# baryshnikova-lab/safepy

Hardware: AMD Instinct MI355X
Metric: node-attribute enrichments/sec (nodes x attrs x perms), compute_pvalues permutation test (higher is better)
Workload: dtype u1 (bit-sliced integer counts; f64 outputs)

## Files before the change

include/safe_hip.h:

```cpp
#ifndef SAFE_HIP_H
#define SAFE_HIP_H

#include <stddef.h>
#include <stdint.h>

#ifdef __cplusplus
extern "C" {
#endif

#define SAFE_HIP_ABI_VERSION 6

#define SAFE_OK 0
#define SAFE_E_INVALID (-1)
#define SAFE_E_HIP (-2)
#define SAFE_E_NOMEM (-3)
#define SAFE_E_UNSUPPORTED (-4)
#define SAFE_E_VALUE (-5)

#define SAFE_DTYPE_F32 0
#define SAFE_DTYPE_F64 1
#define SAFE_DTYPE_U8 2

#define SAFE_SCORE_SUM 0
#define SAFE_SCORE_ZSCORE 1
// ... 84 lines not shown
                             uint64_t key, safe_perms **out);
int safe_ctx_share_stream(safe_ctx *ctx, const char *name, int local_rank, int local_world, int64_t capacity_bytes);
int safe_ctx_unshare_stream(safe_ctx *ctx);
int safe_perms_create_shared(safe_ctx *ctx, int64_t n, const uint8_t *movable_host, int64_t num_permutations,
                             int has_seed, uint32_t seed, safe_perms **out);
int safe_perms_timing(safe_perms *perms, double *out5);
int safe_perms_twin_stats(safe_perms *perms, int *twin_active, int64_t *chunks, int64_t *chunks_won_by_twin);
int safe_ring_open(const char *name, int local_rank, int local_world, int64_t capacity_bytes, safe_ring **out);
int safe_ring_close(safe_ring *ring);
int safe_ring_begin(safe_ring *ring, int64_t n, int64_t k, int64_t count, uint64_t movable_hash, int64_t slot_bytes);
int safe_ring_publish(safe_ring *ring, int64_t chunk, const void *src_host, size_t bytes);
int safe_ring_fetch(safe_ring *ring, int64_t chunk, void *dst_host, size_t bytes);
int safe_ring_end(safe_ring *ring);
int safe_rng_permutations_host(uint32_t seed, const int64_t *values, int64_t n_items,
                               int64_t count, int64_t *out);

int safe_score(safe_ctx *ctx, safe_nbr *nbr, safe_attr *attr, int score_type,
               int64_t col0, int64_t col1, double *out_dev);

int safe_permtest_counts(safe_ctx *ctx, safe_nbr *nbr, safe_attr *attr, safe_perms *perms,
                         int score_type, int64_t col0, int64_t col1, double *ns_dev,
                         double *counts_neg_dev, double *counts_pos_dev);

int safe_randomization(safe_ctx *ctx, safe_nbr *nbr, safe_attr *attr, safe_perms *perms,
                       int score_type, int sign_mode, double enrichment_threshold,
                       const double *nes_table_host, int64_t col0, int64_t col1,
                       double *ns_dev, double *pvalues_neg_dev, double *pvalues_pos_dev,
                       double *nes_dev, double *nes_binary_dev, double *num_enriched_dev);

int safe_hypergeom(safe_ctx *ctx, safe_nbr *nbr, safe_attr *attr, double enrichment_threshold,
// ... 71 lines not shown
```

safepy_amd/_lib.py:

```python
import ctypes as C
import os

_HERE = os.path.dirname(os.path.abspath(__file__))
LIB_PATH = os.path.join(_HERE, 'libsafe_hip.so')

ABI_VERSION = 6
DTYPE_F32, DTYPE_F64, DTYPE_U8 = 0, 1, 2
SCORE_SUM, SCORE_ZSCORE = 0, 1
SIGN_HIGHEST, SIGN_LOWEST, SIGN_BOTH = 0, 1, 2
E_INVALID, E_HIP, E_NOMEM, E_UNSUPPORTED, E_VALUE = -1, -2, -3, -4, -5


class SafeHipError(RuntimeError):
    def __init__(self, code, message):
        super().__init__('libsafe_hip error %d: %s' % (code, message))
        self.code = code


if not os.path.exists(LIB_PATH):
    raise ImportError(
        'safepy_amd: %s not found. Build it with `python -c "import __graft_entry__ as g; g.build()"` or '
        '`make -C safepy_amd/csrc` (needs hipcc, --offload-arch=gfx950). There is no CPU fallback.' % LIB_PATH)


# ... 62 lines not shown
                                     C.POINTER(C.c_int)]),
    'safe_attr_create_host': (C.c_int, [_vp, _vp, C.c_int, _i64, _i64, _i64, _i64, _pp]),
    'safe_attr_create_dev': (C.c_int, [_vp, _vp, C.c_int, _i64, _i64, _i64, _i64, _pp]),
    'safe_attr_destroy': (C.c_int, [_vp]),
    'safe_attr_reindex': (C.c_int, [_vp, _vp, C.c_int, _i64, _i64, _i64, _i64, _vp, _i64, C.c_double, C.c_int, _vp, _pp]),
    'safe_attr_value_counts': (C.c_int, [_vp, _pi64, _pi64, _pi64, _pi64]),
    'safe_attr_nan_to_zero': (C.c_int, [_vp]),
    'safe_attr_download': (C.c_int, [_vp, _vp]),
    'safe_attr_stats': (C.c_int, [_vp, _pi64, _pi64, _pi64, _pi64]),
    'safe_attr_row_flags': (C.c_int, [_vp, _vp]),
    'safe_attr_set_row_flags': (C.c_int, [_vp, _vp]),
    'safe_perms_create': (C.c_int, [_vp, _i64, _vp, _i64, C.c_int, C.c_uint32, _pp]),
    'safe_perms_destroy': (C.c_int, [_vp]),
    'safe_perms_read': (C.c_int, [_vp, _i64, _i64, _vp]),
    'safe_rng_permutations_host': (C.c_int, [C.c_uint32, _vp, _i64, _i64, _vp]),
    'safe_score': (C.c_int, [_vp, _vp, _vp, C.c_int, _i64, _i64, _vp]),
    'safe_permtest_counts': (C.c_int, [_vp, _vp, _vp, _vp, C.c_int, _i64, _i64, _vp, _vp, _vp]),
    'safe_randomization': (C.c_int, [_vp, _vp, _vp, _vp, C.c_int, C.c_int, C.c_double, _vp, _i64, _i64,
                                     _vp, _vp, _vp, _vp, _vp, _vp]),
    'safe_hypergeom': (C.c_int, [_vp, _vp, _vp, C.c_double, _i64, _i64, _vp, _vp, _vp, _vp]),
    'safe_enriched_components': (C.c_int, [_vp, _i64, _i64, _vp, _vp, _vp, _i64, _vp]),
    'safe_jaccard_condensed': (C.c_int, [_vp, _i64, _i64, _vp, _vp]),
    'safe_fdr_adjust': (C.c_int, [_vp, _i64, _i64, _i64, C.c_int, C.c_double, _vp, _vp, _vp, _vp, _vp]),
    'safe_export_packed_counts': (C.c_int, [_vp, _vp, _i64, _pi64, _pi64, C.POINTER(C.c_int)]),
    'safe_nes_from_packed_counts': (C.c_int, [_vp, _vp, _vp, C.c_int, _i64, _i64, _i64, C.c_int, _vp, _vp]),
    'safe_outputs_from_packed_counts': (C.c_int, [_vp, _vp, _vp, C.c_int, _i64, _i64, _i64, C.c_int, C.c_double, _vp, _vp, _vp, _vp, _vp]),
    'safe_set_exchange_chunks': (C.c_int, [_vp, C.c_int, _i64, _vp, _vp]),
    'safe_packed_chunk_info': (C.c_int, [_vp, C.POINTER(C.c_int), _pi64, _pi64]),
    'safe_export_packed_chunk': (C.c_int, [_vp, C.c_int, _vp, _i64, _vp]),
    'safe_export_packed_chunk_narrow': (C.c_int, [_vp, C.c_int, _vp, _i64, _vp]),
# ... 56 lines not shown
```

safepy_amd/backend.py:

```python
import collections
import ctypes as C
import os

import numpy as np

from . import _lib
from ._lib import lib, check

_SCORE = {'sum': _lib.SCORE_SUM, 'z-score': _lib.SCORE_ZSCORE}
_SIGN = {'highest': _lib.SIGN_HIGHEST, 'lowest': _lib.SIGN_LOWEST, 'both': _lib.SIGN_BOTH}


def _ptr(a):
    return C.c_void_p(a.ctypes.data) if a is not None else None


def _split_off_cores(cpus, n_cores, slot=0):
    by_core = {}
    for c in sorted(cpus):
        try:
            sib = set()
            for part in open('/sys/devices/system/cpu/cpu%d/topology/thread_siblings_list' % c).read().strip().split(','):
                lo, _, hi = part.partition('-')
                sib.update(range(int(lo), int(hi or lo) + 1))
# ... 630 lines not shown


def last_mfma_filter(ctx):
    s, u = C.c_int(), C.c_int64()
    check(lib.safe_last_mfma_filter(ctx.handle, C.byref(s), C.byref(u)))
    return s.value, u.value


def rng_permutations_host(seed, values, count):
    values = np.ascontiguousarray(values, dtype=np.int64)
    out = np.empty((count, values.shape[0]), dtype=np.int64)
    check(lib.safe_rng_permutations_host(int(seed), _ptr(values), values.shape[0], int(count), _ptr(out)))
    return out


def nes_table(num_permutations):
    p = np.arange(num_permutations + 1, dtype=np.float64) / num_permutations
    with np.errstate(divide='ignore'):
        return np.ascontiguousarray(-np.log10(np.where(p == 0, 1 / num_permutations, p)))



def score(ctx, nbr, attr, score_type, out_ptr, col0=0, col1=None):
    col1 = attr.m if col1 is None else col1
    check(lib.safe_score(ctx.handle, nbr.handle, attr.handle, _SCORE[score_type], col0, col1, C.c_void_p(out_ptr)))


def permtest_counts(ctx, nbr, attr, perms, score_type, ns_ptr, neg_ptr, pos_ptr, col0=0, col1=None):
    col1 = attr.m if col1 is None else col1
    check(lib.safe_permtest_counts(ctx.handle, nbr.handle, attr.handle, perms.handle, _SCORE[score_type], col0, col1,
# ... 177 lines not shown
```

safepy_amd/csrc/attr.hip:

```cpp
#include "common.h"

template <typename T>
__device__ __forceinline__ double load_attr(const void *raw, int64_t idx) {
    return static_cast<double>(reinterpret_cast<const T *>(raw)[idx]);
}

template <typename T, int GC>
__global__ __launch_bounds__(256) void k_attr_stats(const void *__restrict__ raw, int64_t n, int64_t m,
                                                    int64_t rs, int64_t cs, unsigned int *__restrict__ row_bits,
                                                    unsigned long long *__restrict__ acc ,
                                                    double *__restrict__ col_sum, unsigned long long *__restrict__ max_abs_bits,
                                                    unsigned int *__restrict__ col_nan, int64_t rows_per_block) {
    extern __shared__ unsigned int s_bits[];
    constexpr int RL = 256 / GC;
    const int cx = GC == 1 ? 0 : (threadIdx.x & (GC - 1));
    const int ry = GC == 1 ? threadIdx.x : (threadIdx.x / GC);
    const int lane = threadIdx.x & 63;
    const int64_t j = static_cast<int64_t>(blockIdx.x) * GC + cx;
    const int64_t n_words = (n + 31) / 32;
    __shared__ double s_sum[256];
    __shared__ double s_max[256];
    __shared__ unsigned int s_nan[256], s_other[256], s_nonint[256];
    const int64_t r_begin = static_cast<int64_t>(blockIdx.y) * rows_per_block;
    const int64_t r_end = r_begin + rows_per_block < n ? r_begin + rows_per_block : n;
// ... 310 lines not shown
                       reinterpret_cast<unsigned long long *>(flags + tail_off));
    SAFE_HIP_CHECK(hipGetLastError());
    void *pinned = nullptr;
    SAFE_TRY(ctx_pinned(ctx, flag_bytes, &pinned));
    SAFE_HIP_CHECK(hipMemcpyAsync(pinned, flags, flag_bytes, hipMemcpyDeviceToHost, ctx->stream));
    SAFE_HIP_CHECK(safe_stream_sync(ctx->stream));
    const uint8_t *h_flags = static_cast<const uint8_t *>(pinned);
    unsigned long long h_acc[4];
    memcpy(h_acc, h_flags + tail_off, sizeof(h_acc));
    attr->n_other = static_cast<int64_t>(h_acc[0]);
    attr->max_nan_col = static_cast<int64_t>(h_acc[1]);
    attr->n_non_integer = static_cast<int64_t>(h_acc[2]);
    double mx;
    memcpy(&mx, &h_acc[3], sizeof(double));
    attr->max_abs = mx;
    if (!attr->flags_ready) {
        if (attr->row_flags) ctx_block_free(ctx, attr->row_flags, flag_bytes);
        attr->row_flags = flags;
        attr->flags_ready = true;
        int64_t cnt = 0;
        for (int64_t i = 0; i < n; ++i) cnt += h_flags[i] != 0;
        attr->n_rows_with_value = cnt;
        attr->h_row_flags.assign(h_flags, h_flags + n);
    } else {
        ctx_block_free(ctx, flags, flag_bytes);
    }
    attr->stats_ready = true;
    return SAFE_OK;
}

// ... 264 lines not shown
```

safepy_amd/csrc/common.h:

```cpp
#pragma once
#include <hip/hip_runtime.h>

#include <algorithm>
#include <cstdarg>
#include <cmath>
#include <cstdint>
#include <cstdio>
#include <cstdlib>
#include <cstring>
#include <condition_variable>
#include <mutex>
#include <atomic>
#include <string>
#include <thread>
#include <vector>

#include "safe_hip.h"

#define SAFE_WAVE 64
#define SAFE_PAD_U16 0xFFFFu

void safe_set_error(const char *fmt, ...);
void safe_trace(const char *what);

// ... 59 lines not shown
    int num_cu = 0;
    int64_t hbm_bytes = 0;
    char arch[64] = {0};
    hipEvent_t t0 = nullptr, t1 = nullptr;
    hipEvent_t k0 = nullptr, k1 = nullptr;
    KernelStat last_kernel;
    int last_slices = 0;
    void *diag_prof = nullptr;
    int last_core_slices = 0;
    int64_t last_undecided = 0;
    struct safe_perms *perm_cache = nullptr;
    struct PermRing *ring = nullptr;
    const unsigned int *packed_counts = nullptr;
    int64_t packed_n_pad = 0, packed_m = 0, packed_perms = 0;
    int packed_layout = -1;
    static constexpr int XC_MAX = 8;
    int xc_want = 0;
    int64_t xc_cols = 0;
    void (*xc_callback)(void *) = nullptr;
    void *xc_user = nullptr;
    int xc_made = 0;
    int64_t xc_bounds[XC_MAX + 1] = {};
    int64_t xc_tail_perms = 0;
    hipEvent_t xc_events[XC_MAX] = {};
    std::vector<double> nes_tab_host;
    void *pinned = nullptr;
    size_t pinned_bytes = 0;
    static constexpr int D2H_SLOTS = 8;
    static constexpr size_t D2H_SLOT_BYTES = size_t(4) << 20;
    void *d2h_ring = nullptr;
// ... 71 lines not shown
    int64_t bs_groups = 0;
    int64_t bs_blocks = 0;
    int64_t bs_pieces = 0;
    int64_t bs_src = 0;
    int32_t *bs_order = nullptr;
    int32_t *bs_rowmap = nullptr;
    int32_t *bs_rowcnt = nullptr;
    int32_t *bs_grpmax = nullptr;
    uint4 *bs_bits4p = nullptr;
    int64_t bs_max_group_blocks = 0;
    int32_t *bs_ptr = nullptr;
    int32_t *bs_kb = nullptr;
    uint32_t *bs_bits = nullptr;
    std::vector<int32_t> h_bs_ptr;
    std::vector<int32_t> h_bs_rowmap;
    std::vector<int2> counts_tasks;
    int32_t counts_qoff[9] = {0};
    int64_t counts_tasks_grp = -1;
};

struct HypLookup {
    const int32_t *nid;
    const int32_t *kid;
    const double2 *tab;
    int64_t n_kid, xs;
    double p_cut;
    double *dummy;
    double *pvalues_pos, *nes, *nes_binary;
    unsigned int *enriched;
    unsigned int *cnt16;
// ... 30 lines not shown
    double nes_threshold;
    int sign_mode;
    int mode;
    int64_t ld;
};

struct safe_attr {
    safe_ctx *ctx = nullptr;
    int64_t n = 0, m = 0;
    int dtype = SAFE_DTYPE_F64;
    int64_t row_stride = 0, col_stride = 0;
    const void *raw = nullptr;
    bool owns_raw = false;
    uint8_t *row_flags = nullptr;
    std::vector<uint8_t> h_row_flags;
    bool flags_ready = false;
    bool stats_ready = false;
    int64_t n_other = 0, max_nan_col = 0, n_rows_with_value = 0, n_non_integer = 0;
    double *col_sum = nullptr;
    double max_abs = 0.0;
    int32_t *sup_ptr = nullptr;
    int32_t *sup_row = nullptr;
    int64_t n_ones = 0;
    std::vector<int32_t> h_sup_ptr;
};

struct DrawStream;

struct safe_perms {
    safe_ctx *ctx = nullptr;
// ... 45 lines not shown
    uint16_t *inverse_t = nullptr;
    int64_t inv_stride = 0;
    bool from_table = false;
    bool device_gen = false;
    int32_t *d_movpos = nullptr;
    struct PermRing *ring = nullptr;
    bool ring_consumer = false;
    double t_created_s = 0.0, draw_busy_ms = 0.0, drawn_all_ms = 0.0, enqueued_all_ms = 0.0, ring_wait_ms = 0.0;
};

static inline int64_t ceil_div(int64_t a, int64_t b) { return (a + b - 1) / b; }

int safe_attr_prepare(safe_attr *attr);
int nbr_finalize_from_bits(safe_nbr *nbr);
int nbr_build_transpose(safe_nbr *nbr);
int attr_build_support(safe_attr *attr);
int perms_build_inverse(safe_perms *perms);
int perms_generate_until(safe_perms *perms, int64_t upto);
std::vector<int64_t> perms_stage_plan(int64_t count);
static inline std::vector<int64_t> perm_launch_starts(const safe_perms *perms, int64_t *span, int merge = 1) {
    const int64_t P = perms->count;
    std::vector<int64_t> starts;
    int64_t uniform = 0;
    if (const char *e = getenv("SAFE_HIP_BITS_SPAN")) uniform = std::max<int64_t>(16, atoll(e));
    if (uniform > 0) {
        for (int64_t p = 0; p < P; p += uniform) starts.push_back(p);
    } else {
        const std::vector<int64_t> &plan = perms->stages;
        const int64_t nc = static_cast<int64_t>(plan.size()) - 1;
        for (int64_t c = 0; c < nc; ++c)
// ... 24 lines not shown
```

safepy_amd/csrc/enrich.hip:

```cpp
#include <algorithm>
#include <cmath>
#include <numeric>

#include "common.h"

template <typename T, int BN, int PLANES>
__global__ __launch_bounds__(256) void k_tile_prep(const void *__restrict__ raw, int64_t n, int64_t rs, int64_t cs,
                                                   int64_t col0, int64_t mloc, int64_t n_tiles,
                                                   double *__restrict__ bt) {
    const int64_t idx = static_cast<int64_t>(blockIdx.x) * 256 + threadIdx.x;
    const int64_t total = n_tiles * (n + 1) * BN;
    if (idx >= total) return;
    const int c = static_cast<int>(idx % BN);
    const int64_t row = (idx / BN) % (n + 1);
    const int64_t tile = idx / (static_cast<int64_t>(BN) * (n + 1));
    const int64_t j = tile * BN + c;
    double v = 0.0, v2 = 0.0, nn = 0.0;
    if (row < n && j < mloc) {
        const T x = reinterpret_cast<const T *>(raw)[row * rs + (col0 + j) * cs];
        if (x == x) {
            v = static_cast<double>(x);
            v2 = static_cast<double>(static_cast<T>(x * x));
            nn = 1.0;
        }
// ... 2248 lines not shown
    double ph[5][3] = {}, cls_n[5] = {0, 0, 0, 0, 0};
    for (unsigned int i = 0; i < cnt; ++i) {
        const double nb = static_cast<double>(rec[8 * i + 3] >> 32);
        const int c = nb <= 1 ? 0 : nb <= 7 ? 1 : nb <= 31 ? 2 : nb <= 63 ? 3 : 4;
        ph[c][0] += static_cast<double>(rec[8 * i + 4] - rec[8 * i + 1]);
        ph[c][1] += static_cast<double>(rec[8 * i + 5] - rec[8 * i + 4]);
        ph[c][2] += static_cast<double>(rec[8 * i + 2] - rec[8 * i + 5]);
        cls_n[c] += 1.0;
    }
    for (int c = 0; c < 5; ++c)
        if (cls_work[c] > 0)
            fprintf(stderr, "[blk trace]   slices of %-12s: %.3g block-iterations, %.0f clocks each; %.0f wave-tasks: table %.1f | counting %.1f | flush %.1f kclk each\n",
                    names[c], cls_work[c], cls_busy[c] / cls_work[c], cls_n[c], ph[c][0] / cls_n[c] / 1e3, ph[c][1] / cls_n[c] / 1e3, ph[c][2] / cls_n[c] / 1e3);
}

static int launch_bits(safe_ctx *ctx, safe_nbr *nbr, safe_attr *attr, safe_perms *perms, int64_t col0, int64_t col1,
                       const PermOut &out) {
    const int64_t n = nbr->n, mloc = col1 - col0, n_wg = ceil_div(mloc, 64), P = perms->count;
    const BitsForm form = bits_form(n, nbr->max_count, nbr->sell_col2 != nullptr, 160 * 1024);
    SAFE_REQUIRE(form.kind != BITS_NONE, "launch_bits: no bit-sliced form for %lld nodes with neighborhoods of up to %lld members",
                 static_cast<long long>(n), static_cast<long long>(nbr->max_count));
    const bool blk = form.kind == BITS_BLK, half = form.kind == BITS_PRE32;
    const int wv = blk ? 4 : 16;
    const int id_shift = blk ? 3 : half ? 0 : 1;
    const int64_t n_wgt = half ? 2 * n_wg : n_wg;
    safe_trace("launch_bits: enter");
    uint2 *d_bits = nullptr;
    SAFE_TRY(ctx_scratch(ctx, 1, static_cast<size_t>(n_wg) * (n + 1) * sizeof(uint2), reinterpret_cast<void **>(&d_bits)));
    launch_bits_prep(ctx, attr, col0, mloc, n_wg, d_bits);
    safe_trace("launch_bits: prep launched");
    int64_t span = 1;
    const std::vector<int64_t> starts = perm_launch_starts(perms, &span);
    int64_t n_major = static_cast<int64_t>(starts.size()) - 1, p_split = P, xc_wpc = 0;
    int xc_k = 0;
// ... 189 lines not shown
            const uint16_t *ids_c = d_ids[c % NS];
            void *args[] = {(void *)&n, (void *)&ids_c, (void *)&entries_pad, (void *)&nbr->sell_row, (void *)&nbr->slice_off,
                            (void *)&nbr->slice_width, (void *)&nbr->sell_col2, (void *)&nbr->n_slices, (void *)&d_bits, (void *)&n_tasks,
                            (void *)&d_tasks, (void *)&p_base, (void *)&p_limit, (void *)&queue_c, (void *)&mloc, (void *)&d_gl,
                            (void *)&n_pad, (void *)&out.ns};
            SAFE_HIP_CHECK(hipLaunchKernel(kfn, dim3(grid), dim3(1024), args, lds_T, ks));
        }
        SAFE_HIP_CHECK(hipGetLastError());
        SAFE_HIP_CHECK(hipEventRecord(ev[2 * c + 1], ks));
    }
    ctx->packed_counts = d_gl;
    ctx->packed_n_pad = n_pad;
    ctx->packed_m = mloc;
    ctx->packed_perms = P;
    ctx->packed_layout = 0;
    SAFE_REQUIRE(xc_rc == SAFE_OK, "launch_bits: recording a column chunk's event failed");
    if (n_tail) {
        ctx->xc_made = static_cast<int>(n_tail);
        ctx->xc_tail_perms = tail_span;
        for (int64_t k = 0; k <= n_tail; ++k) ctx->xc_bounds[k] = std::min<int64_t>(k * ctx->xc_cols, mloc);
        ctx->xc_bounds[n_tail] = mloc;
        safe_trace("launch_bits: column chunks enqueued");
        if (ctx->xc_callback) ctx->xc_callback(ctx->xc_user);
    }
    for (int b = 1; b < NS; ++b) {
        SAFE_HIP_CHECK(hipEventRecord(plain[b], kstreams[b]));
        SAFE_HIP_CHECK(hipStreamWaitEvent(ctx->stream, plain[b], 0));
    }
    SAFE_TRY(enrich_finalize_counts(ctx, d_gl, n_pad, nbr->sell_row, mloc, P, out, nullptr));
    SAFE_HIP_CHECK(hipGetLastError());
// ... 358 lines not shown
                 (long long)ctx->packed_perms);
    *c0 = std::min<int64_t>(chunk * ctx->xc_cols, ctx->packed_m);
    *c1 = chunk + 1 == ctx->xc_want ? ctx->packed_m : std::min<int64_t>((chunk + 1) * ctx->xc_cols, ctx->packed_m);
    const int64_t need = (*c1 - *c0) * (narrow ? ctx->packed_n_pad / 8 * 5 : ctx->packed_n_pad);
    SAFE_REQUIRE(capacity >= need, "%s: buffer holds %lld %s, %lld needed", fn, (long long)capacity, narrow ? "words" : "counters", (long long)need);
    SAFE_HIP_CHECK(hipSetDevice(ctx->device));
    *s = stream ? static_cast<hipStream_t>(stream) : ctx->stream;
    if (ctx->xc_made > 0) {
        SAFE_REQUIRE(ctx->xc_made == ctx->xc_want && ctx->xc_bounds[chunk] == *c0 && ctx->xc_bounds[chunk + 1] == *c1,
                     "%s: the call's chunks are not the armed ones", fn);
        SAFE_HIP_CHECK(hipStreamWaitEvent(*s, ctx->xc_events[chunk], 0));
    }
    return SAFE_OK;
}

extern "C" {

int safe_score(safe_ctx *ctx, safe_nbr *nbr, safe_attr *attr, int score_type, int64_t col0, int64_t col1,
               double *out_dev) {
    SAFE_REQUIRE(ctx && out_dev, "safe_score: NULL argument");
    SAFE_TRY(check_cols(nbr, attr, col0, col1, "safe_score"));
    SAFE_REQUIRE(score_type == SAFE_SCORE_SUM || score_type == SAFE_SCORE_ZSCORE, "safe_score: bad score_type %d", score_type);
    SAFE_HIP_CHECK(hipSetDevice(ctx->device));
    const bool z = score_type == SAFE_SCORE_ZSCORE;
    const CountsRoute route = z ? CountsRoute{} : counts_route(route_switches(), nbr, attr);
    if (route.bits) {
        if (route.mfma) {
            HypLookup hl{};
            hl.pvalues_pos = out_dev;
            SAFE_TRY(launch_mfma_counts(ctx, nbr, attr, col0, col1, hl));
// ... 200 lines not shown
    }
    return SAFE_OK;
}

int safe_export_packed_counts(safe_ctx *ctx, uint32_t *dst_dev, int64_t capacity, int64_t *n_pad, int64_t *m,
                              int *layout) {
    SAFE_REQUIRE(ctx && n_pad && m && layout, "safe_export_packed_counts: NULL argument");
    *layout = ctx->packed_layout;
    *n_pad = ctx->packed_layout >= 0 ? ctx->packed_n_pad : 0;
    *m = ctx->packed_layout >= 0 ? ctx->packed_m : 0;
    if (!dst_dev || ctx->packed_layout < 0) return SAFE_OK;
    const int64_t count = ctx->packed_n_pad * ctx->packed_m;
    SAFE_REQUIRE(capacity >= count, "safe_export_packed_counts: buffer holds %lld counters, %lld needed", (long long)capacity,
                 (long long)count);
    SAFE_HIP_CHECK(hipSetDevice(ctx->device));
    SAFE_HIP_CHECK(hipMemcpyAsync(dst_dev, ctx->packed_counts, static_cast<size_t>(count) * sizeof(uint32_t),
                                  hipMemcpyDeviceToDevice, ctx->stream));
    return SAFE_OK;
}

int safe_outputs_from_packed_counts(safe_ctx *ctx, safe_nbr *nbr, const uint32_t *counts_dev, int layout, int64_t n_pad, int64_t m,
                                    int64_t num_permutations, int sign_mode, double enrichment_threshold,
                                    const double *nes_table_host, double *pvalues_neg_dev, double *pvalues_pos_dev,
                                    double *nes_dev, double *nes_binary_dev) {
    SAFE_REQUIRE(ctx && nbr && counts_dev, "safe_outputs_from_packed_counts: NULL argument");
    SAFE_REQUIRE(pvalues_neg_dev || pvalues_pos_dev || nes_dev || nes_binary_dev, "safe_outputs_from_packed_counts: no output requested");
    SAFE_REQUIRE(layout == 0 || layout == 1, "safe_outputs_from_packed_counts: bad layout %d", layout);
    SAFE_REQUIRE(sign_mode >= SAFE_SIGN_HIGHEST && sign_mode <= SAFE_SIGN_BOTH, "safe_outputs_from_packed_counts: bad sign_mode %d", sign_mode);
    SAFE_REQUIRE(num_permutations >= 1 && num_permutations <= 65535 && m >= 1, "safe_outputs_from_packed_counts: bad sizes");
    SAFE_REQUIRE(enrichment_threshold > 0.0 || !nes_binary_dev, "safe_outputs_from_packed_counts: enrichment_threshold must be positive");
    const int32_t *rowmap = layout == 0 ? nbr->sell_row : nbr->bs_rowmap;
    const int64_t want_pad = layout == 0 ? nbr->n_slices * 64 : nbr->bs_groups * 256;
// ... 27 lines not shown
int safe_packed_chunk_info(safe_ctx *ctx, int *chunks, int64_t *bounds, int64_t *tail_permutations) {
    SAFE_REQUIRE(ctx && chunks, "safe_packed_chunk_info: NULL argument");
    const int made = ctx->packed_layout == 0 ? ctx->xc_made : 0;
    *chunks = made;
    if (bounds)
        for (int k = 0; k <= made; ++k) bounds[k] = ctx->xc_bounds[k];
    if (tail_permutations) *tail_permutations = made ? ctx->xc_tail_perms : 0;
    return SAFE_OK;
}

int safe_export_packed_chunk(safe_ctx *ctx, int chunk, uint32_t *dst_dev, int64_t capacity, void *stream) {
    int64_t c0 = 0, c1 = 0;
    hipStream_t s = nullptr;
    SAFE_TRY(packed_chunk_prepare(ctx, chunk, dst_dev, capacity, false, stream, &c0, &c1, &s));
    const int64_t cells = (c1 - c0) * ctx->packed_n_pad;
    if (cells)
        SAFE_HIP_CHECK(hipMemcpyAsync(dst_dev, ctx->packed_counts + c0 * ctx->packed_n_pad, static_cast<size_t>(cells) * sizeof(uint32_t),
                                      hipMemcpyDeviceToDevice, s));
    if (capacity > cells)
        SAFE_HIP_CHECK(hipMemsetAsync(dst_dev + cells, 0, static_cast<size_t>(capacity - cells) * sizeof(uint32_t), s));
    return SAFE_OK;
}

__global__ __launch_bounds__(256) void k_pack_counts20(const unsigned int *__restrict__ counts, int64_t n_pad, int64_t cols,
                                                       unsigned int *__restrict__ dst) {
    const int64_t half = n_pad / 2, idx = static_cast<int64_t>(blockIdx.x) * 256 + threadIdx.x;
    if (idx >= cols * half) return;
    const int64_t c = idx / half, i = idx % half;
    const uint2 v = *reinterpret_cast<const uint2 *>(counts + c * n_pad + 2 * i);
    const unsigned long long x0 = ((v.x >> 16) << 10) | (v.x & 0x3FFu), x1 = ((v.y >> 16) << 10) | (v.y & 0x3FFu);
    const unsigned long long x = x0 | (x1 << 20);
    unsigned int *col = dst + c * (n_pad / 8 * 5);
    col[i] = static_cast<unsigned int>(x);
    reinterpret_cast<unsigned char *>(col + half)[i] = static_cast<unsigned char>(x >> 32);
}

int safe_export_packed_chunk_narrow(safe_ctx *ctx, int chunk, uint32_t *dst_dev, int64_t capacity_words, void *stream) {
    int64_t c0 = 0, c1 = 0;
    hipStream_t s = nullptr;
    SAFE_TRY(packed_chunk_prepare(ctx, chunk, dst_dev, capacity_words, true, stream, &c0, &c1, &s));
    const int64_t words = (c1 - c0) * (ctx->packed_n_pad / 8 * 5);
    if (words) {
        const int64_t pairs = (c1 - c0) * (ctx->packed_n_pad / 2);
        hipLaunchKernelGGL(k_pack_counts20, dim3(static_cast<unsigned int>(ceil_div(pairs, 256))), dim3(256), 0, s,
                           ctx->packed_counts + c0 * ctx->packed_n_pad, ctx->packed_n_pad, c1 - c0, dst_dev);
        SAFE_HIP_CHECK(hipGetLastError());
    }
    if (capacity_words > words)
        SAFE_HIP_CHECK(hipMemsetAsync(dst_dev + words, 0, static_cast<size_t>(capacity_words - words) * sizeof(uint32_t), s));
    return SAFE_OK;
}

int safe_outputs_from_packed_slabs(safe_ctx *ctx, safe_nbr *nbr, const uint32_t *slabs_dev, int layout, int64_t n_pad, int n_slabs,
                                   int64_t slab_stride, const int64_t *slab_cols, const int64_t *out_col0, int64_t m_total,
                                   int64_t num_permutations, int sign_mode, double enrichment_threshold, const double *nes_table_host,
                                   double *pvalues_neg_dev, double *pvalues_pos_dev, double *nes_dev, double *nes_binary_dev,
                                   void *stream) {
    SAFE_REQUIRE(ctx && nbr && slabs_dev && slab_cols && out_col0 && n_slabs >= 1, "safe_outputs_from_packed_slabs: NULL argument");
    SAFE_REQUIRE(pvalues_neg_dev || pvalues_pos_dev || nes_dev || nes_binary_dev, "safe_outputs_from_packed_slabs: no output requested");
    const bool pk20 = (layout & SAFE_PACKED_NARROW) != 0;
// ... 54 lines not shown
```

safepy_amd/csrc/nbr.hip:

```cpp
#include <algorithm>
#include <cmath>
#include <numeric>

#include "common.h"

static double squared_threshold(double nr) {
    if (!(nr > 0.0)) return 0.0;
    if (std::isinf(nr)) return nr;
    double c = nr * nr;
    if (std::isinf(c)) return c;
    while (c > 0.0 && std::sqrt(c) >= nr) c = std::nextafter(c, 0.0);
    while (std::sqrt(c) < nr) c = std::nextafter(c, INFINITY);
    return c;
}

__global__ __launch_bounds__(256) void k_euclid_bits(const double *__restrict__ xy, int64_t n, double thr_sq,
                                                     uint64_t *__restrict__ bits, int64_t words) {
    __shared__ double sx[64], sy[64];
    const int64_t w = blockIdx.x;
    const int64_t i = static_cast<int64_t>(blockIdx.y) * 256 + threadIdx.x;
    const int64_t j0 = w * 64;
    if (threadIdx.x < 64) {
        const int64_t j = j0 + threadIdx.x;
        sx[threadIdx.x] = j < n ? xy[2 * j] : 0.0;
// ... 282 lines not shown
    (void)hipFree(nbr->bits);
    (void)hipFree(nbr->row_ptr);
    (void)hipFree(nbr->col);
    (void)hipFree(nbr->sell_row);
    (void)hipFree(nbr->sell_pos);
    (void)hipFree(nbr->slice_off);
    (void)hipFree(nbr->slice_width);
    (void)hipFree(nbr->sell_col);
    (void)hipFree(nbr->sell_col2);
    (void)hipFree(nbr->sell_col2b);
    (void)hipFree(nbr->dist);
    (void)hipFree(nbr->at_ptr);
    (void)hipFree(nbr->at_col);
    nbr_free_blocks(nbr);
    if (nbr->bits_plan_pinned) (void)hipHostFree(nbr->bits_plan_pinned);
    delete nbr;
}

static int nbr_new(safe_ctx *ctx, int64_t n, safe_nbr **out) {
    SAFE_REQUIRE(n >= 1 && n < (1ll << 31) - 64, "neighborhood size n=%lld out of range", (long long)n);
    safe_nbr *nbr = new safe_nbr();
    nbr->ctx = ctx;
    nbr->n = n;
    nbr->words = ceil_div(n, 64);
    int rc = dev_alloc(&nbr->bits, static_cast<size_t>(n) * nbr->words);
    if (rc != SAFE_OK) {
        nbr_free(nbr);
        return rc;
    }
    *out = nbr;
    return SAFE_OK;
// ... 11 lines not shown
                                  ctx->stream));
    SAFE_HIP_CHECK(safe_stream_sync(ctx->stream));
    (void)hipFree(d_count);

    std::vector<int32_t> row_ptr(n + 1, 0);
    int64_t nnz = 0, max_count = 0;
    for (int64_t i = 0; i < n; ++i) {
        nnz += nbr->h_row_count[i];
        max_count = std::max<int64_t>(max_count, nbr->h_row_count[i]);
        SAFE_REQUIRE(nnz < (1ll << 31), "membership has too many entries for int32 CSR offsets");
        row_ptr[i + 1] = static_cast<int32_t>(nnz);
    }
    nbr->nnz = nnz;
    nbr->max_count = max_count;

    std::vector<int32_t> order(n);
    std::iota(order.begin(), order.end(), 0);
    std::stable_sort(order.begin(), order.end(), [&](int32_t a, int32_t b) {
        return nbr->h_row_count[a] > nbr->h_row_count[b];
    });
    nbr->n_slices = ceil_div(n, 64);
    std::vector<int32_t> sell_row(nbr->n_slices * 64, -1);
    std::copy(order.begin(), order.end(), sell_row.begin());
    std::vector<int32_t> sell_pos(n);
    for (int64_t t = 0; t < n; ++t) sell_pos[order[t]] = static_cast<int32_t>(t);
    nbr->h_slice_width.assign(nbr->n_slices, 0);
    nbr->h_slice_off.assign(nbr->n_slices + 1, 0);
    for (int64_t s = 0; s < nbr->n_slices; ++s) {
        int32_t wdt = nbr->h_row_count[order[s * 64]];
        wdt = (wdt + 7) & ~7;
        nbr->h_slice_width[s] = wdt;
        nbr->h_slice_off[s + 1] = nbr->h_slice_off[s] + static_cast<int64_t>(wdt) * 64;
    }
    nbr->sell_entries = nbr->h_slice_off[nbr->n_slices];

    SAFE_TRY(dev_alloc(&nbr->row_ptr, n + 1));
    SAFE_TRY(dev_alloc(&nbr->col, nnz));
    SAFE_TRY(dev_alloc(&nbr->sell_row, nbr->n_slices * 64));
    SAFE_TRY(dev_alloc(&nbr->sell_pos, n));
    SAFE_HIP_CHECK(hipMemcpyAsync(nbr->sell_pos, sell_pos.data(), n * sizeof(int32_t), hipMemcpyHostToDevice, ctx->stream));
    SAFE_TRY(dev_alloc(&nbr->slice_off, nbr->n_slices + 1));
    SAFE_TRY(dev_alloc(&nbr->slice_width, nbr->n_slices));
    SAFE_TRY(dev_alloc(&nbr->sell_col, nbr->sell_entries));
    SAFE_HIP_CHECK(hipMemcpyAsync(nbr->row_ptr, row_ptr.data(), (n + 1) * sizeof(int32_t), hipMemcpyHostToDevice,
                                  ctx->stream));
    SAFE_HIP_CHECK(hipMemcpyAsync(nbr->sell_row, sell_row.data(), sell_row.size() * sizeof(int32_t),
                                  hipMemcpyHostToDevice, ctx->stream));
    SAFE_HIP_CHECK(hipMemcpyAsync(nbr->slice_off, nbr->h_slice_off.data(), (nbr->n_slices + 1) * sizeof(int64_t),
                                  hipMemcpyHostToDevice, ctx->stream));
    SAFE_HIP_CHECK(hipMemcpyAsync(nbr->slice_width, nbr->h_slice_width.data(), nbr->n_slices * sizeof(int32_t),
                                  hipMemcpyHostToDevice, ctx->stream));
    hipLaunchKernelGGL(k_fill_csr, dim3(ceil_div(n * 64, 256)), dim3(256), 0, ctx->stream, nbr->bits, n, nbr->words,
                       nbr->row_ptr, nbr->col);
    hipLaunchKernelGGL(k_fill_sell, dim3(nbr->n_slices), dim3(64), 0, ctx->stream, nbr->row_ptr, nbr->col,
                       nbr->sell_row, nbr->slice_off, nbr->slice_width, nbr->n_slices, static_cast<int32_t>(n),
                       nbr->sell_col);
    if (n < 32768) {
        const int64_t total = nbr->sell_entries + 1024;
        SAFE_TRY(dev_alloc(&nbr->sell_col2, total));
        hipLaunchKernelGGL(k_sell_scale16, dim3(ceil_div(total, 256)), dim3(256), 0, ctx->stream, nbr->sell_col,
                           nbr->sell_entries, total, static_cast<uint32_t>(2 * n), nbr->sell_col2);
        SAFE_TRY(dev_alloc(&nbr->sell_col2b, total));
        hipLaunchKernelGGL(k_sell_blocked16, dim3(nbr->n_slices + 1), dim3(256), 0, ctx->stream, nbr->sell_col, nbr->slice_off,
                           nbr->slice_width, nbr->n_slices, nbr->sell_entries, total, static_cast<uint32_t>(2 * n),
                           nbr->sell_col2b);
    }
    SAFE_HIP_CHECK(hipGetLastError());
    SAFE_HIP_CHECK(safe_stream_sync(ctx->stream));
    return SAFE_OK;
}

int nbr_build_transpose(safe_nbr *nbr) {
    if (nbr->at_ptr) return SAFE_OK;
    safe_ctx *ctx = nbr->ctx;
    const int64_t n = nbr->n, nnz = nbr->nnz;
    int32_t *d_cnt = nullptr;
    SAFE_TRY(dev_alloc(&d_cnt, n));
    SAFE_HIP_CHECK(hipMemsetAsync(d_cnt, 0, n * sizeof(int32_t), ctx->stream));
    if (nnz) hipLaunchKernelGGL(k_count_cols, dim3(ceil_div(nnz, 256)), dim3(256), 0, ctx->stream, nbr->col, nnz, d_cnt);
    std::vector<int32_t> cnt(n), ptr(n + 1, 0);
    SAFE_HIP_CHECK(hipMemcpyAsync(cnt.data(), d_cnt, n * sizeof(int32_t), hipMemcpyDeviceToHost, ctx->stream));
    SAFE_HIP_CHECK(safe_stream_sync(ctx->stream));
    for (int64_t k = 0; k < n; ++k) ptr[k + 1] = ptr[k] + cnt[k];
// ... 303 lines not shown
    return SAFE_OK;
}

int safe_nbr_csr(safe_nbr *nbr, int32_t *row_ptr_host, int32_t *col_host) {
    SAFE_REQUIRE(nbr && row_ptr_host && col_host, "safe_nbr_csr: NULL argument");
    safe_ctx *ctx = nbr->ctx;
    SAFE_HIP_CHECK(hipSetDevice(ctx->device));
    SAFE_HIP_CHECK(hipMemcpyAsync(row_ptr_host, nbr->row_ptr, (nbr->n + 1) * sizeof(int32_t), hipMemcpyDeviceToHost,
                                  ctx->stream));
    if (nbr->nnz)
        SAFE_HIP_CHECK(hipMemcpyAsync(col_host, nbr->col, nbr->nnz * sizeof(int32_t), hipMemcpyDeviceToHost, ctx->stream));
    SAFE_HIP_CHECK(safe_stream_sync(ctx->stream));
    return SAFE_OK;
}

int safe_nbr_distances(safe_nbr *nbr, double *out_host) {
    SAFE_REQUIRE(nbr && out_host, "safe_nbr_distances: NULL argument");
    SAFE_REQUIRE(nbr->dist != nullptr, "safe_nbr_distances: handle was built without keep_distances");
    safe_ctx *ctx = nbr->ctx;
    SAFE_HIP_CHECK(hipSetDevice(ctx->device));
    SAFE_HIP_CHECK(hipMemcpyAsync(out_host, nbr->dist, nbr->n * nbr->n * sizeof(double), hipMemcpyDeviceToHost,
                                  ctx->stream));
    SAFE_HIP_CHECK(safe_stream_sync(ctx->stream));
    return SAFE_OK;
}

}
```

Before: 5582 billion.

## Drop neighbor entries of rows without attribute values from bit-sliced permutation lists

Builds a filtered SELL neighborhood structure that removes columns for nodes which are neither movable under the permutation nor carry attribute values. Since those nodes contribute zero, the bit-sliced permutation kernel can scan shorter neighbor lists. The filtered slice order differs from the original, so exported counts go through a remap kernel, and the pack-to-20-bit path gathers through the remap. The filtered structure is cached per drop mask; the cost is a one-time host rebuild and an extra indirect gather on export.

Measured after the change: 5709 billion (median of 6 runs). +2.3%, better.

```diff
diff --git a/include/safe_hip.h b/include/safe_hip.h
--- a/include/safe_hip.h
+++ b/include/safe_hip.h
@@ -122,6 +122,8 @@
 int safe_ring_end(safe_ring *ring);
 int safe_rng_permutations_host(uint32_t seed, const int64_t *values, int64_t n_items,
                                int64_t count, int64_t *out);
+int safe_sell_lists_host(int64_t n, const int32_t *row_ptr, const int32_t *col, const uint8_t *drop, int64_t *entries,
+                         int32_t *row_ptr_out, int32_t *col_out, int32_t *sell_row_out);
 
 int safe_score(safe_ctx *ctx, safe_nbr *nbr, safe_attr *attr, int score_type,
                int64_t col0, int64_t col1, double *out_dev);
diff --git a/safepy_amd/_lib.py b/safepy_amd/_lib.py
--- a/safepy_amd/_lib.py
+++ b/safepy_amd/_lib.py
@@ -100,6 +100,7 @@
     'safe_perms_destroy': (C.c_int, [_vp]),
     'safe_perms_read': (C.c_int, [_vp, _i64, _i64, _vp]),
     'safe_rng_permutations_host': (C.c_int, [C.c_uint32, _vp, _i64, _i64, _vp]),
+    'safe_sell_lists_host': (C.c_int, [_i64, _vp, _vp, _vp, _pi64, _vp, _vp, _vp]),
     'safe_score': (C.c_int, [_vp, _vp, _vp, C.c_int, _i64, _i64, _vp]),
     'safe_permtest_counts': (C.c_int, [_vp, _vp, _vp, _vp, C.c_int, _i64, _i64, _vp, _vp, _vp]),
     'safe_randomization': (C.c_int, [_vp, _vp, _vp, _vp, C.c_int, C.c_int, C.c_double, _vp, _i64, _i64,
diff --git a/safepy_amd/backend.py b/safepy_amd/backend.py
--- a/safepy_amd/backend.py
+++ b/safepy_amd/backend.py
@@ -668,6 +668,20 @@
     return out
 
 
+def sell_lists_host(row_ptr, col, drop=None):
+    row_ptr = np.ascontiguousarray(row_ptr, dtype=np.int32)
+    col = np.ascontiguousarray(col, dtype=np.int32)
+    n = row_ptr.shape[0] - 1
+    drop = None if drop is None else np.ascontiguousarray(drop, dtype=np.uint8)
+    entries = C.c_int64()
+    ptr_out = np.empty(n + 1, dtype=np.int32)
+    col_out = np.empty(max(col.shape[0], 1), dtype=np.int32)
+    sell_row = np.empty(-(-n // 64) * 64, dtype=np.int32)
+    check(lib.safe_sell_lists_host(n, _ptr(row_ptr), _ptr(col), _ptr(drop), C.byref(entries), _ptr(ptr_out), _ptr(col_out),
+                                   _ptr(sell_row)))
+    return {'entries': entries.value, 'row_ptr': ptr_out, 'col': col_out[:ptr_out[-1]], 'sell_row': sell_row}
+
+
 def nes_table(num_permutations):
     p = np.arange(num_permutations + 1, dtype=np.float64) / num_permutations
     with np.errstate(divide='ignore'):
diff --git a/safepy_amd/csrc/attr.hip b/safepy_amd/csrc/attr.hip
--- a/safepy_amd/csrc/attr.hip
+++ b/safepy_amd/csrc/attr.hip
@@ -348,6 +348,7 @@
     double mx;
     memcpy(&mx, &h_acc[3], sizeof(double));
     attr->max_abs = mx;
+    attr->h_local_flags.assign(h_flags, h_flags + n);
     if (!attr->flags_ready) {
         if (attr->row_flags) ctx_block_free(ctx, attr->row_flags, flag_bytes);
         attr->row_flags = flags;
diff --git a/safepy_amd/csrc/common.h b/safepy_amd/csrc/common.h
--- a/safepy_amd/csrc/common.h
+++ b/safepy_amd/csrc/common.h
@@ -97,6 +97,7 @@
     const unsigned int *packed_counts = nullptr;
     int64_t packed_n_pad = 0, packed_m = 0, packed_perms = 0;
     int packed_layout = -1;
+    const int32_t *packed_remap = nullptr;
     static constexpr int XC_MAX = 8;
     int xc_want = 0;
     int64_t xc_cols = 0;
@@ -198,6 +199,9 @@
     uint32_t *bs_bits = nullptr;
     std::vector<int32_t> h_bs_ptr;
     std::vector<int32_t> h_bs_rowmap;
+    safe_nbr *movable_lists = nullptr;
+    std::vector<uint8_t> movable_drop;
+    int32_t *movable_remap = nullptr;
     std::vector<int2> counts_tasks;
     int32_t counts_qoff[9] = {0};
     int64_t counts_tasks_grp = -1;
@@ -258,6 +262,7 @@
     bool owns_raw = false;
     uint8_t *row_flags = nullptr;
     std::vector<uint8_t> h_row_flags;
+    std::vector<uint8_t> h_local_flags;
     bool flags_ready = false;
     bool stats_ready = false;
     int64_t n_other = 0, max_nan_col = 0, n_rows_with_value = 0, n_non_integer = 0;
@@ -333,6 +338,7 @@
 int safe_attr_prepare(safe_attr *attr);
 int nbr_finalize_from_bits(safe_nbr *nbr);
 int nbr_build_transpose(safe_nbr *nbr);
+int nbr_movable_lists(safe_nbr *nbr, const std::vector<uint8_t> &drop, safe_nbr **out);
 int attr_build_support(safe_attr *attr);
 int perms_build_inverse(safe_perms *perms);
 int perms_generate_until(safe_perms *perms, int64_t upto);
diff --git a/safepy_amd/csrc/enrich.hip b/safepy_amd/csrc/enrich.hip
--- a/safepy_amd/csrc/enrich.hip
+++ b/safepy_amd/csrc/enrich.hip
@@ -2286,10 +2286,24 @@
                     names[c], cls_work[c], cls_busy[c] / cls_work[c], cls_n[c], ph[c][0] / cls_n[c] / 1e3, ph[c][1] / cls_n[c] / 1e3, ph[c][2] / cls_n[c] / 1e3);
 }
 
-static int launch_bits(safe_ctx *ctx, safe_nbr *nbr, safe_attr *attr, safe_perms *perms, int64_t col0, int64_t col1,
+static int bits_lists(safe_nbr *nbr, safe_attr *attr, const safe_perms *perms, safe_nbr **out) {
+    *out = nbr;
+    const int64_t n = nbr->n;
+    if (perms->from_table || perms->n != n || perms->k == n || static_cast<int64_t>(perms->h_movable.size()) != perms->k) return SAFE_OK;
+    SAFE_TRY(safe_attr_prepare(attr));
+    if (static_cast<int64_t>(attr->h_local_flags.size()) != n) return SAFE_OK;
+    std::vector<uint8_t> drop(n);
+    for (int64_t i = 0; i < n; ++i) drop[i] = attr->h_local_flags[i] ? 0 : 1;
+    for (const int32_t r : perms->h_movable) drop[r] = 0;
+    return nbr_movable_lists(nbr, drop, out);
+}
+
+static int launch_bits(safe_ctx *ctx, safe_nbr *nbr_full, safe_attr *attr, safe_perms *perms, int64_t col0, int64_t col1,
                        const PermOut &out) {
+    safe_nbr *nbr = nullptr;
+    SAFE_TRY(bits_lists(nbr_full, attr, perms, &nbr));
     const int64_t n = nbr->n, mloc = col1 - col0, n_wg = ceil_div(mloc, 64), P = perms->count;
-    const BitsForm form = bits_form(n, nbr->max_count, nbr->sell_col2 != nullptr, 160 * 1024);
+    const BitsForm form = bits_form(n, nbr_full->max_count, nbr_full->sell_col2 != nullptr, 160 * 1024);
     SAFE_REQUIRE(form.kind != BITS_NONE, "launch_bits: no bit-sliced form for %lld nodes with neighborhoods of up to %lld members",
                  static_cast<long long>(n), static_cast<long long>(nbr->max_count));
     const bool blk = form.kind == BITS_BLK, half = form.kind == BITS_PRE32;
@@ -2509,6 +2523,7 @@
     ctx->packed_m = mloc;
     ctx->packed_perms = P;
     ctx->packed_layout = 0;
+    ctx->packed_remap = nbr != nbr_full ? nbr->movable_remap : nullptr;
     SAFE_REQUIRE(xc_rc == SAFE_OK, "launch_bits: recording a column chunk's event failed");
     if (n_tail) {
         ctx->xc_made = static_cast<int>(n_tail);
@@ -2897,6 +2912,26 @@
     return SAFE_OK;
 }
 
+__global__ __launch_bounds__(256) void k_counts_remap(const unsigned int *__restrict__ counts, const int32_t *__restrict__ remap,
+                                                      int64_t n_pad, int64_t cols, unsigned int *__restrict__ dst) {
+    const int64_t idx = static_cast<int64_t>(blockIdx.x) * 256 + threadIdx.x;
+    if (idx >= cols * n_pad) return;
+    dst[idx] = counts[(idx / n_pad) * n_pad + remap[idx % n_pad]];
+}
+
+static int copy_packed_columns(safe_ctx *ctx, int64_t c0, int64_t c1, uint32_t *dst_dev, hipStream_t s) {
+    const int64_t cells = (c1 - c0) * ctx->packed_n_pad;
+    const unsigned int *src = ctx->packed_counts + c0 * ctx->packed_n_pad;
+    if (ctx->packed_layout == 0 && ctx->packed_remap) {
+        hipLaunchKernelGGL(k_counts_remap, dim3(static_cast<unsigned int>(ceil_div(cells, 256))), dim3(256), 0, s, src, ctx->packed_remap,
+                           ctx->packed_n_pad, c1 - c0, dst_dev);
+        SAFE_HIP_CHECK(hipGetLastError());
+    } else {
+        SAFE_HIP_CHECK(hipMemcpyAsync(dst_dev, src, static_cast<size_t>(cells) * sizeof(uint32_t), hipMemcpyDeviceToDevice, s));
+    }
+    return SAFE_OK;
+}
+
 extern "C" {
 
 int safe_score(safe_ctx *ctx, safe_nbr *nbr, safe_attr *attr, int score_type, int64_t col0, int64_t col1,
@@ -3127,8 +3162,7 @@
     SAFE_REQUIRE(capacity >= count, "safe_export_packed_counts: buffer holds %lld counters, %lld needed", (long long)capacity,
                  (long long)count);
     SAFE_HIP_CHECK(hipSetDevice(ctx->device));
-    SAFE_HIP_CHECK(hipMemcpyAsync(dst_dev, ctx->packed_counts, static_cast<size_t>(count) * sizeof(uint32_t),
-                                  hipMemcpyDeviceToDevice, ctx->stream));
+    SAFE_TRY(copy_packed_columns(ctx, 0, ctx->packed_m, dst_dev, ctx->stream));
     return SAFE_OK;
 }
 
@@ -3186,20 +3220,19 @@
     hipStream_t s = nullptr;
     SAFE_TRY(packed_chunk_prepare(ctx, chunk, dst_dev, capacity, false, stream, &c0, &c1, &s));
     const int64_t cells = (c1 - c0) * ctx->packed_n_pad;
-    if (cells)
-        SAFE_HIP_CHECK(hipMemcpyAsync(dst_dev, ctx->packed_counts + c0 * ctx->packed_n_pad, static_cast<size_t>(cells) * sizeof(uint32_t),
-                                      hipMemcpyDeviceToDevice, s));
+    if (cells) SAFE_TRY(copy_packed_columns(ctx, c0, c1, dst_dev, s));
     if (capacity > cells)
         SAFE_HIP_CHECK(hipMemsetAsync(dst_dev + cells, 0, static_cast<size_t>(capacity - cells) * sizeof(uint32_t), s));
     return SAFE_OK;
 }
 
-__global__ __launch_bounds__(256) void k_pack_counts20(const unsigned int *__restrict__ counts, int64_t n_pad, int64_t cols,
-                                                       unsigned int *__restrict__ dst) {
+__global__ __launch_bounds__(256) void k_pack_counts20(const unsigned int *__restrict__ counts, const int32_t *__restrict__ remap,
+                                                       int64_t n_pad, int64_t cols, unsigned int *__restrict__ dst) {
     const int64_t half = n_pad / 2, idx = static_cast<int64_t>(blockIdx.x) * 256 + threadIdx.x;
     if (idx >= cols * half) return;
     const int64_t c = idx / half, i = idx % half;
-    const uint2 v = *reinterpret_cast<const uint2 *>(counts + c * n_pad + 2 * i);
+    const unsigned int *col_in = counts + c * n_pad;
+    const uint2 v = remap ? make_uint2(col_in[remap[2 * i]], col_in[remap[2 * i + 1]]) : *reinterpret_cast<const uint2 *>(col_in + 2 * i);
     const unsigned long long x0 = ((v.x >> 16) << 10) | (v.x & 0x3FFu), x1 = ((v.y >> 16) << 10) | (v.y & 0x3FFu);
     const unsigned long long x = x0 | (x1 << 20);
     unsigned int *col = dst + c * (n_pad / 8 * 5);
@@ -3215,7 +3248,8 @@
     if (words) {
         const int64_t pairs = (c1 - c0) * (ctx->packed_n_pad / 2);
         hipLaunchKernelGGL(k_pack_counts20, dim3(static_cast<unsigned int>(ceil_div(pairs, 256))), dim3(256), 0, s,
-                           ctx->packed_counts + c0 * ctx->packed_n_pad, ctx->packed_n_pad, c1 - c0, dst_dev);
+                           ctx->packed_counts + c0 * ctx->packed_n_pad, ctx->packed_layout == 0 ? ctx->packed_remap : nullptr,
+                           ctx->packed_n_pad, c1 - c0, dst_dev);
         SAFE_HIP_CHECK(hipGetLastError());
     }
     if (capacity_words > words)
diff --git a/safepy_amd/csrc/nbr.hip b/safepy_amd/csrc/nbr.hip
--- a/safepy_amd/csrc/nbr.hip
+++ b/safepy_amd/csrc/nbr.hip
@@ -320,7 +320,77 @@
     (void)hipFree(nbr->at_col);
     nbr_free_blocks(nbr);
     if (nbr->bits_plan_pinned) (void)hipHostFree(nbr->bits_plan_pinned);
+    (void)hipFree(nbr->movable_remap);
+    nbr_free(nbr->movable_lists);
     delete nbr;
+}
+
+static void sell_slices(const std::vector<int32_t> &count, std::vector<int32_t> &sell_row, std::vector<int32_t> &sell_pos,
+                        std::vector<int32_t> &slice_width, std::vector<int64_t> &slice_off) {
+    const int64_t n = static_cast<int64_t>(count.size()), n_slices = ceil_div(n, 64);
+    std::vector<int32_t> order(n);
+    std::iota(order.begin(), order.end(), 0);
+    std::stable_sort(order.begin(), order.end(), [&](int32_t a, int32_t b) { return count[a] > count[b]; });
+    sell_row.assign(n_slices * 64, -1);
+    std::copy(order.begin(), order.end(), sell_row.begin());
+    sell_pos.resize(n);
+    for (int64_t t = 0; t < n; ++t) sell_pos[order[t]] = static_cast<int32_t>(t);
+    slice_width.assign(n_slices, 0);
+    slice_off.assign(n_slices + 1, 0);
+    for (int64_t s = 0; s < n_slices; ++s) {
+        const int32_t wdt = (count[order[s * 64]] + 7) & ~7;
+        slice_width[s] = wdt;
+        slice_off[s + 1] = slice_off[s] + static_cast<int64_t>(wdt) * 64;
+    }
+}
+
+static void csr_without_rows(int64_t n, const int32_t *row_ptr, const int32_t *col, const uint8_t *drop, std::vector<int32_t> &out_ptr,
+                             std::vector<int32_t> &out_col) {
+    out_ptr.assign(n + 1, 0);
+    out_col.clear();
+    out_col.reserve(row_ptr[n]);
+    for (int64_t i = 0; i < n; ++i) {
+        for (int32_t e = row_ptr[i]; e < row_ptr[i + 1]; ++e)
+            if (!drop[col[e]]) out_col.push_back(col[e]);
+        out_ptr[i + 1] = static_cast<int32_t>(out_col.size());
+    }
+}
+
+static int nbr_build_sell(safe_nbr *nbr) {
+    safe_ctx *ctx = nbr->ctx;
+    const int64_t n = nbr->n;
+    std::vector<int32_t> sell_row, sell_pos;
+    sell_slices(nbr->h_row_count, sell_row, sell_pos, nbr->h_slice_width, nbr->h_slice_off);
+    nbr->n_slices = ceil_div(n, 64);
+    nbr->sell_entries = nbr->h_slice_off[nbr->n_slices];
+    SAFE_TRY(dev_alloc(&nbr->sell_row, nbr->n_slices * 64));
+    SAFE_TRY(dev_alloc(&nbr->sell_pos, n));
+    SAFE_HIP_CHECK(hipMemcpyAsync(nbr->sell_pos, sell_pos.data(), n * sizeof(int32_t), hipMemcpyHostToDevice, ctx->stream));
+    SAFE_TRY(dev_alloc(&nbr->slice_off, nbr->n_slices + 1));
+    SAFE_TRY(dev_alloc(&nbr->slice_width, nbr->n_slices));
+    SAFE_TRY(dev_alloc(&nbr->sell_col, nbr->sell_entries));
+    SAFE_HIP_CHECK(hipMemcpyAsync(nbr->sell_row, sell_row.data(), sell_row.size() * sizeof(int32_t),
+                                  hipMemcpyHostToDevice, ctx->stream));
+    SAFE_HIP_CHECK(hipMemcpyAsync(nbr->slice_off, nbr->h_slice_off.data(), (nbr->n_slices + 1) * sizeof(int64_t),
+                                  hipMemcpyHostToDevice, ctx->stream));
+    SAFE_HIP_CHECK(hipMemcpyAsync(nbr->slice_width, nbr->h_slice_width.data(), nbr->n_slices * sizeof(int32_t),
+                                  hipMemcpyHostToDevice, ctx->stream));
+    hipLaunchKernelGGL(k_fill_sell, dim3(nbr->n_slices), dim3(64), 0, ctx->stream, nbr->row_ptr, nbr->col,
+                       nbr->sell_row, nbr->slice_off, nbr->slice_width, nbr->n_slices, static_cast<int32_t>(n),
+                       nbr->sell_col);
+    if (n < 32768) {
+        const int64_t total = nbr->sell_entries + 1024;
+        SAFE_TRY(dev_alloc(&nbr->sell_col2, total));
+        hipLaunchKernelGGL(k_sell_scale16, dim3(ceil_div(total, 256)), dim3(256), 0, ctx->stream, nbr->sell_col,
+                           nbr->sell_entries, total, static_cast<uint32_t>(2 * n), nbr->sell_col2);
+        SAFE_TRY(dev_alloc(&nbr->sell_col2b, total));
+        hipLaunchKernelGGL(k_sell_blocked16, dim3(nbr->n_slices + 1), dim3(256), 0, ctx->stream, nbr->sell_col, nbr->slice_off,
+                           nbr->slice_width, nbr->n_slices, nbr->sell_entries, total, static_cast<uint32_t>(2 * n),
+                           nbr->sell_col2b);
+    }
+    SAFE_HIP_CHECK(hipGetLastError());
+    SAFE_HIP_CHECK(safe_stream_sync(ctx->stream));
+    return SAFE_OK;
 }
 
 static int nbr_new(safe_ctx *ctx, int64_t n, safe_nbr **out) {
@@ -362,59 +432,78 @@
     nbr->nnz = nnz;
     nbr->max_count = max_count;
 
-    std::vector<int32_t> order(n);
-    std::iota(order.begin(), order.end(), 0);
-    std::stable_sort(order.begin(), order.end(), [&](int32_t a, int32_t b) {
-        return nbr->h_row_count[a] > nbr->h_row_count[b];
-    });
-    nbr->n_slices = ceil_div(n, 64);
-    std::vector<int32_t> sell_row(nbr->n_slices * 64, -1);
-    std::copy(order.begin(), order.end(), sell_row.begin());
-    std::vector<int32_t> sell_pos(n);
-    for (int64_t t = 0; t < n; ++t) sell_pos[order[t]] = static_cast<int32_t>(t);
-    nbr->h_slice_width.assign(nbr->n_slices, 0);
-    nbr->h_slice_off.assign(nbr->n_slices + 1, 0);
-    for (int64_t s = 0; s < nbr->n_slices; ++s) {
-        int32_t wdt = nbr->h_row_count[order[s * 64]];
-        wdt = (wdt + 7) & ~7;
-        nbr->h_slice_width[s] = wdt;
-        nbr->h_slice_off[s + 1] = nbr->h_slice_off[s] + static_cast<int64_t>(wdt) * 64;
-    }
-    nbr->sell_entries = nbr->h_slice_off[nbr->n_slices];
-
     SAFE_TRY(dev_alloc(&nbr->row_ptr, n + 1));
     SAFE_TRY(dev_alloc(&nbr->col, nnz));
-    SAFE_TRY(dev_alloc(&nbr->sell_row, nbr->n_slices * 64));
-    SAFE_TRY(dev_alloc(&nbr->sell_pos, n));
-    SAFE_HIP_CHECK(hipMemcpyAsync(nbr->sell_pos, sell_pos.data(), n * sizeof(int32_t), hipMemcpyHostToDevice, ctx->stream));
-    SAFE_TRY(dev_alloc(&nbr->slice_off, nbr->n_slices + 1));
-    SAFE_TRY(dev_alloc(&nbr->slice_width, nbr->n_slices));
-    SAFE_TRY(dev_alloc(&nbr->sell_col, nbr->sell_entries));
     SAFE_HIP_CHECK(hipMemcpyAsync(nbr->row_ptr, row_ptr.data(), (n + 1) * sizeof(int32_t), hipMemcpyHostToDevice,
                                   ctx->stream));
-    SAFE_HIP_CHECK(hipMemcpyAsync(nbr->sell_row, sell_row.data(), sell_row.size() * sizeof(int32_t),
-                                  hipMemcpyHostToDevice, ctx->stream));
-    SAFE_HIP_CHECK(hipMemcpyAsync(nbr->slice_off, nbr->h_slice_off.data(), (nbr->n_slices + 1) * sizeof(int64_t),
-                                  hipMemcpyHostToDevice, ctx->stream));
-    SAFE_HIP_CHECK(hipMemcpyAsync(nbr->slice_width, nbr->h_slice_width.data(), nbr->n_slices * sizeof(int32_t),
-                                  hipMemcpyHostToDevice, ctx->stream));
     hipLaunchKernelGGL(k_fill_csr, dim3(ceil_div(n * 64, 256)), dim3(256), 0, ctx->stream, nbr->bits, n, nbr->words,
                        nbr->row_ptr, nbr->col);
-    hipLaunchKernelGGL(k_fill_sell, dim3(nbr->n_slices), dim3(64), 0, ctx->stream, nbr->row_ptr, nbr->col,
-                       nbr->sell_row, nbr->slice_off, nbr->slice_width, nbr->n_slices, static_cast<int32_t>(n),
-                       nbr->sell_col);
-    if (n < 32768) {
-        const int64_t total = nbr->sell_entries + 1024;
-        SAFE_TRY(dev_alloc(&nbr->sell_col2, total));
-        hipLaunchKernelGGL(k_sell_scale16, dim3(ceil_div(total, 256)), dim3(256), 0, ctx->stream, nbr->sell_col,
-                           nbr->sell_entries, total, static_cast<uint32_t>(2 * n), nbr->sell_col2);
-        SAFE_TRY(dev_alloc(&nbr->sell_col2b, total));
-        hipLaunchKernelGGL(k_sell_blocked16, dim3(nbr->n_slices + 1), dim3(256), 0, ctx->stream, nbr->sell_col, nbr->slice_off,
-                           nbr->slice_width, nbr->n_slices, nbr->sell_entries, total, static_cast<uint32_t>(2 * n),
-                           nbr->sell_col2b);
-    }
-    SAFE_HIP_CHECK(hipGetLastError());
+    return nbr_build_sell(nbr);
+}
+
+static int nbr_build_without_rows(safe_nbr *nbr, const std::vector<uint8_t> &drop, safe_nbr **out) {
+    safe_ctx *ctx = nbr->ctx;
+    const int64_t n = nbr->n, n_pad = nbr->n_slices * 64;
+    *out = nullptr;
+    std::vector<int32_t> row_ptr(n + 1), col(nbr->nnz), unf_row(n_pad);
+    SAFE_HIP_CHECK(hipMemcpyAsync(row_ptr.data(), nbr->row_ptr, (n + 1) * sizeof(int32_t), hipMemcpyDeviceToHost, ctx->stream));
+    if (nbr->nnz)
+        SAFE_HIP_CHECK(hipMemcpyAsync(col.data(), nbr->col, nbr->nnz * sizeof(int32_t), hipMemcpyDeviceToHost, ctx->stream));
+    SAFE_HIP_CHECK(hipMemcpyAsync(unf_row.data(), nbr->sell_row, n_pad * sizeof(int32_t), hipMemcpyDeviceToHost, ctx->stream));
     SAFE_HIP_CHECK(safe_stream_sync(ctx->stream));
+    std::vector<int32_t> f_ptr, f_col;
+    csr_without_rows(n, row_ptr.data(), col.data(), drop.data(), f_ptr, f_col);
+    safe_nbr *f = new safe_nbr();
+    f->ctx = ctx;
+    f->n = n;
+    f->words = nbr->words;
+    f->nnz = static_cast<int64_t>(f_col.size());
+    f->h_row_count.resize(n);
+    for (int64_t i = 0; i < n; ++i) {
+        f->h_row_count[i] = f_ptr[i + 1] - f_ptr[i];
+        f->max_count = std::max<int64_t>(f->max_count, f->h_row_count[i]);
+    }
+    int rc = dev_alloc(&f->row_ptr, n + 1);
+    if (rc == SAFE_OK) rc = dev_alloc(&f->col, f->nnz);
+    if (rc == SAFE_OK && (hipMemcpyAsync(f->row_ptr, f_ptr.data(), (n + 1) * sizeof(int32_t), hipMemcpyHostToDevice, ctx->stream) != hipSuccess ||
+                          (f->nnz && hipMemcpyAsync(f->col, f_col.data(), f->nnz * sizeof(int32_t), hipMemcpyHostToDevice, ctx->stream) != hipSuccess))) {
+        safe_set_error("nbr_build_without_rows: upload failed");
+        rc = SAFE_E_HIP;
+    }
+    if (rc == SAFE_OK) rc = nbr_build_sell(f);
+    if (rc == SAFE_OK) {
+        std::vector<int32_t> f_row, f_pos, remap(n_pad), f_width;
+        std::vector<int64_t> f_off;
+        sell_slices(f->h_row_count, f_row, f_pos, f_width, f_off);
+        for (int64_t u = 0; u < n_pad; ++u) remap[u] = unf_row[u] >= 0 ? f_pos[unf_row[u]] : static_cast<int32_t>(u);
+        rc = dev_alloc(&f->movable_remap, n_pad);
+        if (rc == SAFE_OK && (hipMemcpyAsync(f->movable_remap, remap.data(), n_pad * sizeof(int32_t), hipMemcpyHostToDevice, ctx->stream) != hipSuccess ||
+                              safe_stream_sync(ctx->stream) != hipSuccess)) {
+            safe_set_error("nbr_build_without_rows: upload failed");
+            rc = SAFE_E_HIP;
+        }
+    }
+    if (rc != SAFE_OK) {
+        nbr_free(f);
+        return rc;
+    }
+    *out = f;
+    return SAFE_OK;
+}
+
+int nbr_movable_lists(safe_nbr *nbr, const std::vector<uint8_t> &drop, safe_nbr **out) {
+    *out = nbr;
+    if (std::find(drop.begin(), drop.end(), uint8_t(1)) == drop.end()) return SAFE_OK;
+    if (nbr->movable_lists && nbr->movable_drop == drop) {
+        *out = nbr->movable_lists;
+        return SAFE_OK;
+    }
+    nbr_free(nbr->movable_lists);
+    nbr->movable_lists = nullptr;
+    nbr->movable_drop.clear();
+    SAFE_TRY(nbr_build_without_rows(nbr, drop, &nbr->movable_lists));
+    nbr->movable_drop = drop;
+    *out = nbr->movable_lists;
     return SAFE_OK;
 }
 
@@ -748,6 +837,22 @@
     return SAFE_OK;
 }
 
+int safe_sell_lists_host(int64_t n, const int32_t *row_ptr, const int32_t *col, const uint8_t *drop, int64_t *entries,
+                         int32_t *row_ptr_out, int32_t *col_out, int32_t *sell_row_out) {
+    SAFE_REQUIRE(n >= 1 && row_ptr && col && entries, "safe_sell_lists_host: bad argument");
+    std::vector<int32_t> f_ptr(row_ptr, row_ptr + n + 1), f_col(col, col + row_ptr[n]);
+    if (drop) csr_without_rows(n, row_ptr, col, drop, f_ptr, f_col);
+    std::vector<int32_t> count(n), sell_row, sell_pos, width;
+    std::vector<int64_t> off;
+    for (int64_t i = 0; i < n; ++i) count[i] = f_ptr[i + 1] - f_ptr[i];
+    sell_slices(count, sell_row, sell_pos, width, off);
+    *entries = off.back();
+    if (row_ptr_out) std::copy(f_ptr.begin(), f_ptr.end(), row_ptr_out);
+    if (col_out) std::copy(f_col.begin(), f_col.end(), col_out);
+    if (sell_row_out) std::copy(sell_row.begin(), sell_row.end(), sell_row_out);
+    return SAFE_OK;
+}
+
 int safe_nbr_distances(safe_nbr *nbr, double *out_host) {
     SAFE_REQUIRE(nbr && out_host, "safe_nbr_distances: NULL argument");
     SAFE_REQUIRE(nbr->dist != nullptr, "safe_nbr_distances: handle was built without keep_distances");
```
